# city96/ComfyUI-GGUF

Measured on NVIDIA H100. Metric: standalone dequant throughput, GGUF packed -> fp16 (algorithmic GB/s = packed bytes read + output bytes written), higher is better.
Workload: dtype f16

## Files before the change

### comfyui-gguf_b200/csrc/api.cu

```cuda
#include <stdlib.h>

#include "blocks.cuh"
#include "fallback.cuh"
#include "internal.h"

using namespace ggufb200;

static bool type_geom(int t, int *bs, int *ts)
{
    int b = 1, s = 2;
    const bool known = t == T_BF16 || with_block(t, false, [&](auto blk) {
        b = decltype(blk)::BS;
        s = decltype(blk)::TS;
        return true;
    });
    if (!known) return false;
    if (bs) *bs = b;
    if (ts) *ts = s;
    return true;
}

static bool dtype_ok(int d) { return d >= 0 && d <= 2; }
static bool aligned16(const void *p) { return (reinterpret_cast<uintptr_t>(p) & 15) == 0; }
static bool fused_type(int t) { return t != T_BF16 && type_geom(t, nullptr, nullptr); }

static int device_check()
{
    static signed char ok[64] = {};
    int dev = 0;
    if (cudaGetDevice(&dev) != cudaSuccess) {
        cudaGetLastError();
        return GGUFB200_E_CUDA;
    }
    if (dev < 0 || dev >= 64) return GGUFB200_OK;
    if (ok[dev] == 0) {
        int major = 0, minor = 0;
        if (cudaDeviceGetAttribute(&major, cudaDevAttrComputeCapabilityMajor, dev) != cudaSuccess ||
            cudaDeviceGetAttribute(&minor, cudaDevAttrComputeCapabilityMinor, dev) != cudaSuccess) {
            cudaGetLastError();
            return GGUFB200_E_CUDA;
        }
        ok[dev] = (major == 9 && minor == 0) ? 1 : -1;
    }
    return ok[dev] == 1 ? GGUFB200_OK : GGUFB200_E_DEVICE;
}

struct Route {
    int algo;
    size_t ws;
};

static LinearOptions linear_options(int flags, bool straddled)
{
    LinearOptions o;
    if (flags & GGUFB200_FLAG_GENERIC) o.producers = LinearOptions::GENERIC;
    else if (flags & GGUFB200_FLAG_EXACT_W) o.producers = LinearOptions::EXACT;
    if (flags & GGUFB200_FLAG_TILE384) o.tile = 384;
    else if (flags & GGUFB200_FLAG_TILE192) o.tile = 192;
    o.nosplit = (flags & GGUFB200_FLAG_NOSPLIT) != 0 || straddled;
    return o;
}

static Route pick_route(int type, const void *W, long long M, long long N, long long K, int act, int math, int algo_flags,
                        const LinearOptions &opt, size_t ws_avail, bool have_spans = false)
{
    const int algo = algo_flags & GGUFB200_ALGO_MASK;
    const int flags = algo_flags & ~GGUFB200_ALGO_MASK;
    const size_t dense = (size_t)N * (size_t)K * 2;
    const bool w_ok = !W || aligned16(W);
    int bs = 1;
    type_geom(type, &bs, nullptr);
    const bool straddled = straddled_rows(bs, N, K);
    const bool fusable = fused_type(type) && math == kF16 && (K % 64) == 0 && (N % 8) == 0 && !straddled;
    Route r{algo, 0};
    if (algo == GGUFB200_ALGO_AUTO) {
        const bool tmem_ok = w_ok && fused_type(type) && math == kF16 && (N % 8) == 0 && (have_spans || fused_tmem_supported(type, W, N, K));
        const bool exact = (flags & GGUFB200_FLAG_EXACT_W) != 0 || math != kF16;
        if (!w_ok) r.algo = GGUFB200_ALGO_DEQUANT_MMA;
        else if (straddled) r.algo = GGUFB200_ALGO_DEQUANT_MMA;
        else if (M <= gemv_max_m() && !exact && gemv2_supported(type, W ? W : (const void *)16, N, K, M)) r.algo = GGUFB200_ALGO_GEMV_FAST;
        else if (M <= gemv_max_m()) r.algo = GGUFB200_ALGO_GEMV;
        else if (tmem_ok) r.algo = GGUFB200_ALGO_FUSED_TMEM;
        else if (fusable && ws_avail < dense) r.algo = GGUFB200_ALGO_FUSED_MMA;
        else r.algo = GGUFB200_ALGO_DEQUANT_MMA;
    }
    switch (r.algo) {
    case GGUFB200_ALGO_DEQUANT_MMA: r.ws = dense; break;
    case GGUFB200_ALGO_FUSED_MMA: r.ws = fusable ? fused_mma_workspace(M, N, K, opt) : 0; break;
    case GGUFB200_ALGO_FUSED_TMEM: r.ws = fused_tmem_workspace(M, N, K, opt); break;
    default: r.ws = 0;
    }
    (void)act;
    return r;
}

extern "C" {

int ggufb200_version(void) { return GGUFB200_VERSION; }

const char *ggufb200_strerror(int rc)
{
    switch (rc) {
    case GGUFB200_OK: return "ok";
    case GGUFB200_E_TYPE: return "unsupported ggml quantization type (no CPU fallback is provided)";
    case GGUFB200_E_DTYPE: return "dtype code must be 0 (float16), 1 (bfloat16) or 2 (float32)";
    case GGUFB200_E_ALIGN: return "output / activation pointers must be 16-byte aligned";
    case GGUFB200_E_SHAPE: return "bad shape: sizes must be non-negative, K a multiple of the block size (or of 8 with N*K a multiple of a 256-element block), ld >= row length";
    case GGUFB200_E_NULL: return "required pointer is NULL";
    case GGUFB200_E_CUDA: return "CUDA launch failed";
    case GGUFB200_E_WORKSPACE: return "workspace too small (see ggufb200_linear_workspace)";
    case GGUFB200_E_UNSUPPORTED: return "operation not implemented for this type / dtype / shape combination";
    case GGUFB200_E_DEVICE: return "current CUDA device is not sm_90 (H100)";
// ... 349 lines not shown
```

### comfyui-gguf_b200/csrc/dequant.cu

```cuda
#include <type_traits>

#include "blocks.cuh"
#include "fallback.cuh"
#include "internal.h"
#include "wgmma.cuh"

namespace ggufb200 {

constexpr int kThreads = 128;

int g_dequant_pdl = 1;

__device__ __forceinline__ void st_otile_v4(uint32_t saddr, uint32_t a, uint32_t b, uint32_t c, uint32_t d)
{
    asm volatile("st.shared.v4.b32 [%0], {%1, %2, %3, %4};" ::"r"(saddr), "r"(a), "r"(b), "r"(c), "r"(d));
}

template <class Q, int MATH, int OUT>
__device__ __forceinline__ void dequant_tile(const uint8_t *tile, uint8_t *otile, int tile_elems, int tid)
{
    constexpr int OB = OutT<OUT>::bytes;
    constexpr int EPC = 16 / OB;
    constexpr int CH = 32 / EPC;
    const int blk_in_tile = (tid * 32) / Q::BS;
    const int e0 = (tid * 32) % Q::BS;
    if constexpr (IsFallback<Q>::value) {
        static_assert(MATH == kF32, "the fallback formats are decoded in fp32 only");
        if (tid * 32 < tile_elems) {
            float v[32];
            Q::run32(tile + blk_in_tile * Q::TS, e0, v);
            const uint32_t obase = smem_u32(otile) + tid * (32 * OB);
            const uint32_t sw = (obase >> 7) & (CH - 1);
#pragma unroll
            for (int c = 0; c < CH; ++c) {
                const float *f = v + c * EPC;
                const uint32_t oaddr = obase + ((uint32_t)c ^ sw) * 16;
                if constexpr (OUT == kF32) {
                    st_otile_v4(oaddr, __float_as_uint(f[0]), __float_as_uint(f[1]), __float_as_uint(f[2]), __float_as_uint(f[3]));
                } else {
                    st_otile_v4(oaddr, pack16<OUT, kF32>(make_float2(f[0], f[1])), pack16<OUT, kF32>(make_float2(f[2], f[3])),
                                pack16<OUT, kF32>(make_float2(f[4], f[5])), pack16<OUT, kF32>(make_float2(f[6], f[7])));
                }
            }
        }
    } else {
        constexpr int GROUP = GroupOf<Q>::value;
        if (tid * 32 < tile_elems) {
            const uint8_t *blk = tile + blk_in_tile * Q::TS;
            const GroupScale<MATH> g0 = group_scale<Q, MATH>(blk, e0);
            GroupScale<MATH> g1 = g0;
            if constexpr (GROUP == 16) g1 = group_scale<Q, MATH>(blk, e0 + 16);
            const uint32_t obase = smem_u32(otile) + tid * (32 * OB);
            const uint32_t sw = (obase >> 7) & (CH - 1);
#pragma unroll
            for (int c = 0; c < CH; ++c) {
                const int e = e0 + c * EPC;
                const bool second = (GROUP == 16) && (c * EPC >= 16);
                typename Math<MATH>::T2 v[EPC / 2];
                dequant_elems<Q, MATH, EPC>(blk, e, second ? g1 : g0, v);
                const uint32_t oaddr = obase + ((uint32_t)c ^ sw) * 16;
                if constexpr (OUT == kF32) {
                    float2 f0 = Math<MATH>::to_f32x2(v[0]), f1 = Math<MATH>::to_f32x2(v[1]);
// ... 468 lines not shown
```

### comfyui-gguf_b200/csrc/internal.h

```cpp
#pragma once
#include <cuda_runtime.h>
#include <stddef.h>
#include <stdint.h>

#include "../../include/ggufb200.h"

namespace ggufb200 {

extern int g_dequant_pdl;
extern int g_gemv2_ctas;

int dequant_dispatch(int type, const void *packed, long long n_blocks, void *out, int out_dtype, int math_dtype, cudaStream_t st, bool stable = false);
int fallback_dispatch(int type, const void *packed, long long n_blocks, void *out, int out_dtype, cudaStream_t st, bool stable);
int unpack_dispatch(int type, const void *packed, long long n_blocks, int16_t *q, int16_t *sc, int16_t *mn, cudaStream_t st);
int rows_dispatch(int type, const void *packed, long long n_table_rows, long long K, const long long *rows, long long n_rows, void *out,
                  int out_dtype, int math_dtype, cudaStream_t st);
constexpr int kKronMaxPatches = 8;
int dequant_kron_dispatch(int type, const void *packed, long long N, long long K, void *out, int out_dtype, int math_dtype,
                          const ggufb200_kron_patch *patches, int n_patches, cudaStream_t st, bool stable);
constexpr int kLowrankMaxPatches = GGUFB200_LOWRANK_MAX_PATCHES;
int dequant_lowrank_dispatch(int type, const void *packed, long long N, long long K, void *out, int out_dtype, int math_dtype,
                             const ggufb200_lowrank_patch *patches, int n_patches, cudaStream_t st);

int gemv_max_m();
int gemv_dispatch(int type, const void *W, long long N, long long K, const void *X, long long M, long long ldx, int act_dtype, int math_dtype,
                  const void *bias, int bias_dtype, void *Y, long long ldy, cudaStream_t st);
bool gemv2_supported(int type, const void *W, long long N, long long K, long long M);
int gemv2_dispatch(int type, const void *W, long long N, long long K, const void *X, long long M, long long ldx, int act_dtype, const void *bias,
                   int bias_dtype, void *Y, long long ldy, cudaStream_t st, bool w_stable = false);

inline bool straddled_rows(int block_size, long long N, long long K)
{
    return block_size == 256 && K % 256 != 0 && (N * K) % 256 == 0;
}

size_t repack_bytes(int type, long long N, long long K, int *pitch, long long *span_stride);
int repack_dispatch(int type, const void *W, long long N, long long K, void *out, cudaStream_t st);

struct LinearOptions {
    enum Producers { FAST, EXACT, GENERIC };
    Producers producers = FAST;
    int tile = 0;
    bool nosplit = false;
};

int dense_gemm(const void *W, long long N, long long K, long long ldw, const void *X, long long M, long long ldx, int act_dtype,
               const void *bias, int bias_dtype, void *Y, long long ldy, cudaStream_t st, const float *scale = nullptr);
size_t fused_mma_workspace(long long M, long long N, long long K, const LinearOptions &opt);
void fused_mma_plan(long long M, long long N, long long K, size_t ws_bytes, const LinearOptions &opt, int *tile_rows, int *splits,
                    int *kb_per_split, int *ctas);
int fused_mma_linear(int type, const void *W, long long N, long long K, const void *X, long long M, long long ldx, int act_dtype,
                     const void *bias, int bias_dtype, void *Y, long long ldy, void *ws, size_t ws_bytes, const LinearOptions &opt,
                     cudaStream_t st);
constexpr int kLoraMaxKblocks = 8;
struct LoraOperands {
    const void *T;
    long long ldt;
    const void *U;
    long long ldu;
    int kblocks;
    const int32_t *tiles;
};
bool fused_tmem_supported(int type, const void *W, long long N, long long K);
size_t fused_tmem_workspace(long long M, long long N, long long K, const LinearOptions &opt);
void fused_tmem_plan(long long M, long long N, long long K, size_t ws_bytes, const LinearOptions &opt, int *tile_tokens, int *splits,
                     int *spans_per_split, int *items);
int fused_tmem_linear(int type, const void *W, const void *Wspan, long long span_stride, long long N, long long K, const void *X, long long M,
                      long long ldx, int act_dtype, const void *bias, int bias_dtype, void *Y, long long ldy, void *ws, size_t ws_bytes,
                      const LinearOptions &opt, const LoraOperands &lora, cudaStream_t st, const float *scale = nullptr);

int scale_columns_dispatch(const void *X, long long M, long long K, long long ldx, int act_dtype, const float *col_scale, void *Y,
                           long long ldy, cudaStream_t st);

}
```

### comfyui-gguf_b200/csrc/linear_sm90.cu

```cuda
#include "internal.h"
#include "linear_sm90.cuh"

namespace ggufb200 {

constexpr size_t kSplitWsCap = 24u << 20;
constexpr int kSpan = 256;

static size_t split_ws(size_t ws_bytes) { return ws_bytes > kSplitWsCap ? kSplitWsCap : ws_bytes; }

struct KRanges {
    long long per, count;
};
static KRanges k_ranges(long long spans, long long s)
{
    const long long per = (spans + s - 1) / s;
    return {per, (spans + per - 1) / per};
}

static size_t partial_bytes(int splits, long long M, long long N) { return splits > 1 ? (size_t)splits * (size_t)M * (size_t)N * 4 : 0; }

template <int ACT, int BN, bool SCALED>
static int dense_launch(const void *W, long long N, long long K, long long ldw, const void *X, long long M, long long ldx, const void *bias,
                        int bias_dtype, void *Y, long long ldy, cudaStream_t st, const float *scale)
{
// ... 150 lines not shown
            if (r.count != s) continue;
            const int per = (int)r.per, splits = (int)r.count;
            const long long items = tiles * splits;
            const long long ctas = items * 2 * cands[c].accs;
            const long long rounds = (ctas + sms - 1) / sms;
            const double t_kb = 4.0 * cands[c].tt > 2000.0 ? 4.0 * cands[c].tt : 2000.0;
            double cost = (double)rounds * (4.0 * per * t_kb + 3000.0);
            if (splits > 1) cost += (double)(splits + 1) * (double)slice / (16.0 * sms) + 6000.0;
            if (best.n_items == 0 || cost < best_cost * 0.98) {
                best_cost = cost;
                best.tt = cands[c].tt; best.accs = cands[c].accs; best.splits = splits; best.spans_per_split = per;
                best.ttiles = ttiles; best.ftiles = ftiles; best.n_items = (int)items;
            }
        }
    }
    return best;
}

size_t fused_tmem_workspace(long long M, long long N, long long K, const LinearOptions &opt)
{
    return partial_bytes(tmem_plan(M, N, K, kSplitWsCap, opt.tile, !opt.nosplit).splits, M, N);
}

void fused_tmem_plan(long long M, long long N, long long K, size_t ws_bytes, const LinearOptions &opt, int *tile_tokens, int *splits,
                     int *spans_per_split, int *items)
{
    const TmemPlan pl = tmem_plan(M, N, K, ws_bytes, opt.tile, !opt.nosplit);
    *tile_tokens = pl.tt * pl.accs;
    *splits = pl.splits;
    *spans_per_split = pl.spans_per_split;
    *items = pl.n_items;
}

struct TmemArgs {
    const void *W;
    const void *Wspan;
    long long span_stride;
    long long N, K;
    const void *X;
    long long M, ldx;
    const void *bias;
    int bias_dtype;
    void *Y;
    long long ldy;
    void *ws;
    size_t ws_bytes;
    const LinearOptions &opt;
    const LoraOperands &lora;
    cudaStream_t st;
    bool straddled;
    const float *scale;
};

template <class Q, class Prod, int ACT, int TT, bool SCALED>
static int tmem_launch(const TmemArgs &a, const TmemPlan &pl, float *partial)
{
    CUtensorMap tmX, tmT;
    if (!make_kblock_map(&tmX, a.X, a.M, a.K, a.ldx, ACT, TT)) return GGUFB200_E_CUDA;
    tmT = tmX;
    if (a.lora.T && !make_kblock_map(&tmT, a.lora.T, a.M, (long long)kBlockK * a.lora.kblocks, a.lora.ldt, ACT, TT)) return GGUFB200_E_CUDA;
    WgParams p{};
    p.M = a.M; p.N = a.N; p.K = a.K;
    p.bias = partial ? nullptr : a.bias;
    p.bias_dtype = a.bias_dtype;
    p.Y = reinterpret_cast<uint8_t *>(a.Y);
    p.ldy = a.ldy;
    p.partial = partial;
    p.W = reinterpret_cast<const uint8_t *>(a.W);
    if (a.straddled) {
        p.Wspan = reinterpret_cast<const uint8_t *>(a.Wspan ? a.Wspan : a.W);
        p.span_stride = a.Wspan ? a.span_stride : Q::TS;
    } else {
        p.row_bytes = a.K / Q::BS * Q::TS;
        p.Wspan = reinterpret_cast<const uint8_t *>(a.Wspan);
        p.span_stride = a.span_stride;
    }
    p.loraU = a.lora.T ? reinterpret_cast<const uint16_t *>(a.lora.U) : nullptr;
    p.ldu = a.lora.ldu;
    p.lora_kb = a.lora.kblocks;
    p.lora_tiles = a.lora.tiles;
    p.scale = partial ? nullptr : a.scale;
    p.ftiles = 2 * pl.ftiles;
    p.ttiles = pl.ttiles * pl.accs;
    p.kb_per_split = 4 * pl.spans_per_split;
    p.kb_total = a.straddled ? (int)(a.K / kBlockK) : 4 * (int)((a.K + kSpan - 1) / kSpan);
    if constexpr (Q::BS == 256) {
        if (a.straddled) return wg_launch<Q, Prod, ACT, TT, true, true, SCALED>(tmX, tmX, tmT, p, pl.splits, a.st);
    }
    return wg_launch<Q, Prod, ACT, TT, true, false, SCALED>(tmX, tmX, tmT, p, pl.splits, a.st);
}

template <class Q, class Prod, int ACT, bool SCALED> static int tmem_tiles(const TmemArgs &a, const TmemPlan &pl, float *partial)
{
    if (pl.tt == 32) return tmem_launch<Q, Prod, ACT, 32, SCALED>(a, pl, partial);
    if (pl.tt == 128) return tmem_launch<Q, Prod, ACT, 128, SCALED>(a, pl, partial);
    return tmem_launch<Q, Prod, ACT, 192, SCALED>(a, pl, partial);
}

template <class Q> struct FmaMatters {
    static constexpr bool value = Q::TS == 144 || Q::TS == 176;
};

template <class Q, int ACT, bool SCALED> static int tmem_run(const TmemArgs &a)
{
    const TmemPlan pl = tmem_plan(a.M, a.N, a.K, a.ws_bytes, a.opt.tile, !a.opt.nosplit);
    float *partial = pl.splits > 1 ? reinterpret_cast<float *>(a.ws) : nullptr;
    int rc;
    if constexpr (!FastProducer<Q>::fast) {
        rc = tmem_tiles<Q, Producer<Q>, ACT, SCALED>(a, pl, partial);
    } else if (a.opt.producers == LinearOptions::GENERIC) {
        rc = tmem_tiles<Q, Producer<Q>, ACT, SCALED>(a, pl, partial);
    } else if constexpr (FmaMatters<Q>::value) {
        rc = a.opt.producers == LinearOptions::EXACT ? tmem_tiles<Q, FastProducer<Q, false>, ACT, SCALED>(a, pl, partial)
                                                     : tmem_tiles<Q, FastProducer<Q, true>, ACT, SCALED>(a, pl, partial);
    } else {
        rc = tmem_tiles<Q, FastProducer<Q, true>, ACT, SCALED>(a, pl, partial);
    }
    if (rc != GGUFB200_OK || !partial) return rc;
    return wg_finalize<ACT, SCALED>(partial, pl.splits, a.bias, a.bias_dtype, a.Y, a.M, a.N, a.ldy, a.st, a.scale);
}

template <class Q> static bool canonical_ok(const void *W, long long N, long long K)
{
    const bool aligned = SpanOf<Q>::BYTES % 16 == 0 && K % kBlockK == 0 && (reinterpret_cast<uintptr_t>(W) & 15) == 0;
    if (straddled_rows(Q::BS, N, K)) return aligned;
    return aligned && (K / Q::BS * Q::TS) % 16 == 0;
}

bool fused_tmem_supported(int type, const void *W, long long N, long long K)
{
    if (N % 8 != 0 || K % 8 != 0) return false;
    return with_block(type, false, [&](auto blk) { return canonical_ok<decltype(blk)>(W, N, K); });
}

int fused_tmem_linear(int type, const void *W, const void *Wspan, long long span_stride, long long N, long long K, const void *X, long long M,
                      long long ldx, int act_dtype, const void *bias, int bias_dtype, void *Y, long long ldy, void *ws, size_t ws_bytes,
                      const LinearOptions &opt, const LoraOperands &lora, cudaStream_t st, const float *scale)
{
    if (N % 8 != 0 || K % 8 != 0) return GGUFB200_E_UNSUPPORTED;
    return with_block(type, GGUFB200_E_UNSUPPORTED, [&](auto blk) {
        using Q = decltype(blk);
        const bool straddled = straddled_rows(Q::BS, N, K);
// ... 10 lines not shown
```

### comfyui-gguf_b200/csrc/linear_sm90.cuh

```cuda
#pragma once
#include <type_traits>

#include "produce.cuh"
#include "wgmma.cuh"

namespace ggufb200 {

constexpr int kWgThreads = 384;

struct WgParams {
    long long M, N, K;
    const void *bias;
    int bias_dtype;
    uint8_t *Y;
    long long ldy;
    float *partial;
    const uint8_t *W;
    long long row_bytes;
    const uint8_t *Wspan;
    long long span_stride;
    const uint16_t *loraU;
    int ttiles, ftiles;
    int kb_per_split, kb_total;
    long long ldu;
    int lora_kb;
    const int *lora_tiles;
    const float *scale;
};

template <int TN, bool TRANS> struct WgCfg {
    static constexpr int TOK = TRANS ? TN : 128;
    static constexpr int FEAT = TRANS ? 128 : TN;
    static constexpr int A_BYTES = 128 * 128;
    static constexpr int B_BYTES = TN * 128;
    static constexpr int STAGE = A_BYTES + B_BYTES;
    static constexpr int RAW_STAGES = (227 * 1024 - 2048) / STAGE;
    static constexpr int STAGES = RAW_STAGES > 8 ? 8 : RAW_STAGES;
    static constexpr int YPITCH = FEAT * 2 + 16;
    static constexpr int SMEM = STAGES * STAGE + 1024 + 256;
    static_assert(TOK * YPITCH <= STAGES * STAGE, "epilogue staging reuses the operand ring");
    static_assert(B_BYTES % 1024 == 0, "swizzled tiles need 1024-byte alignment");
};

template <int ACT> __device__ __forceinline__ uint32_t wg_h2_to_act(uint32_t h)
{
    if constexpr (ACT == kBF16) {
        const float2 f = __half22float2(*reinterpret_cast<const __half2 *>(&h));
        const __nv_bfloat162 b = __floats2bfloat162_rn(f.x, f.y);
        return *reinterpret_cast<const uint32_t *>(&b);
    } else {
        return h;
    }
}

template <class Q, class Prod, int ACT, int TN, bool TRANS, bool STRADDLED = false, bool SCALED = false>
__global__ void __launch_bounds__(kWgThreads, 1)
wg_linear_kernel(const __grid_constant__ CUtensorMap tmX, const __grid_constant__ CUtensorMap tmW, const __grid_constant__ CUtensorMap tmT,
                 const WgParams p)
{
    using Cfg = WgCfg<TN, TRANS>;
    constexpr bool DENSE = std::is_same<Prod, void>::value;
    constexpr int STAGES = Cfg::STAGES, TOK = Cfg::TOK, FEAT = Cfg::FEAT;
    constexpr int WROWS = TRANS ? 128 : TN;

    const int per = p.ftiles * p.ttiles;
    const int split = blockIdx.x / per;
    const int rem = blockIdx.x - split * per;
    const long long feat0 = (long long)(rem / p.ttiles) * FEAT;
    const long long tok0 = (long long)(rem % p.ttiles) * TOK;
    if (tok0 >= p.M || feat0 >= p.N) return;
    const int kb0 = split * p.kb_per_split;
    const int nkb_main = min(p.kb_per_split, p.kb_total - kb0);
    int lora_first = 0, lora_n = 0;
    if (p.loraU != nullptr && split == 0) {
        lora_n = p.lora_kb;
        if (p.lora_tiles) {
            const long long ft = feat0 / 128;
            lora_first = min(max(p.lora_tiles[2 * ft], 0), p.lora_kb);
            lora_n = min(max(p.lora_tiles[2 * ft + 1], 0), p.lora_kb - lora_first);
        }
    }
    const int nkb = nkb_main + lora_n;

    extern __shared__ uint8_t wg_smem_raw[];
    uint8_t *tiles = reinterpret_cast<uint8_t *>((reinterpret_cast<uintptr_t>(wg_smem_raw) + 1023) & ~(uintptr_t)1023);
    uint64_t *full = reinterpret_cast<uint64_t *>(tiles + STAGES * Cfg::STAGE);
    uint64_t *empty = full + STAGES;

    const int wg = threadIdx.x >> 7;
    const int t = threadIdx.x & 127;
    if (threadIdx.x == 0) {
        for (int s = 0; s < STAGES; ++s) {
            mbar_init(&full[s], DENSE ? 1 : 1 + 4);
            mbar_init(&empty[s], 256);
        }
        fence_mbar_init();
    }
    __syncthreads();

    if (wg == 0) {
        for (int i = 0; i < nkb; ++i) {
            const int s = i % STAGES;
            mbar_wait(&empty[s], (uint32_t)(((i / STAGES) & 1) ^ 1));
            uint8_t *a_tile = tiles + s * Cfg::STAGE;
            uint8_t *b_tile = a_tile + Cfg::A_BYTES;
            uint8_t *x_tile = TRANS ? b_tile : a_tile;
            uint8_t *w_tile = TRANS ? a_tile : b_tile;
            const int kb = kb0 + i;
            const bool lora_kb = i >= nkb_main;
            const int lj = lora_first + i - nkb_main;
            if (t == 0) {
                mbar_arrive_expect_tx(&full[s], TOK * 128 + (DENSE ? WROWS * 128 : 0));
                tma_load_2d(x_tile, lora_kb ? &tmT : &tmX, &full[s], lora_kb ? lj * kBlockK : kb * kBlockK, (int)tok0);
                if constexpr (DENSE) tma_load_2d(w_tile, &tmW, &full[s], kb * kBlockK, (int)feat0);
            }
            if constexpr (!DENSE) {
#pragma unroll 1
                for (int r = t; r < WROWS; r += 128) {
                    const long long n = feat0 + r;
                    const uint32_t dst = smem_u32(w_tile) + (uint32_t)r * 128;
                    auto emit = [&](int half, const uint32_t (&o)[16]) {
#pragma unroll
                        for (int c = 0; c < 4; ++c) {
                            const int chunk = half * 4 + c;
                            st_shared_v4(dst + (uint32_t)((chunk ^ (r & 7)) << 4), wg_h2_to_act<ACT>(o[4 * c]), wg_h2_to_act<ACT>(o[4 * c + 1]),
                                         wg_h2_to_act<ACT>(o[4 * c + 2]), wg_h2_to_act<ACT>(o[4 * c + 3]));
                        }
                    };
                    if (n >= p.N || (!lora_kb && (long long)kb * kBlockK >= p.K)) {
#pragma unroll
                        for (int c = 0; c < 8; ++c) st_shared_v4(dst + (uint32_t)(c << 4), 0, 0, 0, 0);
                    } else if (lora_kb) {
                        const uint4 *urow = reinterpret_cast<const uint4 *>(p.loraU + n * p.ldu + lj * kBlockK);
#pragma unroll
                        for (int half = 0; half < 2; ++half) {
                            uint32_t o[16];
#pragma unroll
                            for (int q = 0; q < 4; ++q) {
                                const uint4 v = urow[half * 4 + q];
                                o[4 * q] = v.x; o[4 * q + 1] = v.y; o[4 * q + 2] = v.z; o[4 * q + 3] = v.w;
                            }
                            emit(half, o);
                        }
                    } else if constexpr (STRADDLED) {
                        static_assert(TRANS && Q::BS == 256, "straddled rows: FUSED_TMEM, 256-element blocks");
                        const long long e = n * p.K + (long long)kb * kBlockK;
                        Prod::run64(p.Wspan + (e >> 8) * p.span_stride, (int)(e >> 6) & 3, emit);
                    } else {
                        const int span = kb >> 2;
                        const uint8_t *src = p.Wspan ? p.Wspan + (long long)span * p.span_stride + n * SpanOf<Q>::PITCH
                                                     : p.W + n * p.row_bytes + (long long)span * SpanOf<Q>::BYTES;
                        Prod::run64(src, kb & 3, emit);
                    }
                }
                fence_proxy_async_smem();
                __syncwarp();
                if ((t & 31) == 0) mbar_arrive(&full[s]);
            }
        }
        return;
    }

    const int cw = wg - 1;
    constexpr int NR = TN / 2;
    float acc[NR];
#pragma unroll
    for (int j = 0; j < NR; ++j) acc[j] = 0.f;
    const uint32_t base = smem_u32(tiles);
    for (int i = 0; i < nkb; ++i) {
        const int s = i % STAGES;
        mbar_wait(&full[s], (uint32_t)((i / STAGES) & 1));
        const uint32_t a_addr = base + (uint32_t)(s * Cfg::STAGE) + (uint32_t)(cw * 64 * 128);
        const uint32_t b_addr = base + (uint32_t)(s * Cfg::STAGE + Cfg::A_BYTES);
        const uint64_t da = wg_desc_sw128(a_addr), db = wg_desc_sw128(b_addr);
        wgmma_fence();
#pragma unroll
        for (int j = 0; j < kBlockK / 16; ++j) Wgmma<ACT, TN>::mma(acc, da + (uint64_t)(2 * j), db + (uint64_t)(2 * j));
        wgmma_commit();
        if (i > 0) {
            wgmma_wait<1>();
            mbar_arrive(&empty[(i - 1) % STAGES]);
        }
    }
    wgmma_wait<0>();

    const int warp = (threadIdx.x >> 5) & 3, lane = threadIdx.x & 31;
    const int arow0 = cw * 64 + warp * 16 + (lane >> 2);
    const int bcol0 = 2 * (lane & 3);
    if (p.partial) {
        float *P = p.partial + (long long)split * p.M * p.N;
#pragma unroll
        for (int j = 0; j < NR / 4; ++j)
#pragma unroll
            for (int h = 0; h < 2; ++h)
#pragma unroll
                for (int e = 0; e < 2; ++e) {
                    const int ar = arow0 + 8 * h, bc = 8 * j + bcol0 + e;
                    const long long tok = tok0 + (TRANS ? bc : ar), f = feat0 + (TRANS ? ar : bc);
                    if (tok < p.M && f < p.N) P[tok * p.N + f] = acc[4 * j + 2 * h + e];
                }
        return;
    }
    asm volatile("bar.sync 1, 256;" ::: "memory");
    const uint32_t ystage = base;
#pragma unroll
    for (int j = 0; j < NR / 4; ++j)
#pragma unroll
        for (int h = 0; h < 2; ++h)
#pragma unroll
            for (int e = 0; e < 2; ++e) {
                const int ar = arow0 + 8 * h, bc = 8 * j + bcol0 + e;
                const int tk = TRANS ? bc : ar, f = TRANS ? ar : bc;
                float v = acc[4 * j + 2 * h + e];
                if constexpr (SCALED) {
                    if (feat0 + f < p.N) v *= p.scale[feat0 + f];
                }
                if (p.bias && feat0 + f < p.N) v += wg_bias<ACT>(p.bias, p.bias_dtype, feat0 + f);
                uint16_t hb;
                if constexpr (ACT == kBF16) hb = __bfloat16_as_ushort(__float2bfloat16_rn(v));
                else hb = __half_as_ushort(__float2half_rn(v));
                asm volatile("st.shared.u16 [%0], %1;" ::"r"(ystage + (uint32_t)(tk * Cfg::YPITCH + f * 2)), "h"(hb) : "memory");
            }
    asm volatile("bar.sync 1, 256;" ::: "memory");
    constexpr int CPR = FEAT / 8;
    for (int c = threadIdx.x - 128; c < TOK * CPR; c += 256) {
        const int tk = c / CPR, f = (c % CPR) * 8;
        const long long m = tok0 + tk, n = feat0 + f;
        if (m < p.M && n < p.N) {
            uint32_t a, b, cc, d;
            asm volatile("ld.shared.v4.b32 {%0, %1, %2, %3}, [%4];" : "=r"(a), "=r"(b), "=r"(cc), "=r"(d) : "r"(ystage + (uint32_t)(tk * Cfg::YPITCH + f * 2)));
            st_global_v4(p.Y + (m * p.ldy + n) * 2, a, b, cc, d);
        }
    }
}

template <class Q, class Prod, int ACT, int TN, bool TRANS, bool STRADDLED = false, bool SCALED = false>
static int wg_launch(const CUtensorMap &tmX, const CUtensorMap &tmW, const CUtensorMap &tmT, const WgParams &p, int splits, cudaStream_t st)
{
    using Cfg = WgCfg<TN, TRANS>;
    auto kern = wg_linear_kernel<Q, Prod, ACT, TN, TRANS, STRADDLED, SCALED>;
    static unsigned char attr[64] = {};
    if (!ensure_dynamic_smem(kern, Cfg::SMEM, attr)) return GGUFB200_E_CUDA;
    const long long ctas = (long long)p.ftiles * p.ttiles * splits;
    if (ctas <= 0 || ctas > 0x7fffffffll) return GGUFB200_E_SHAPE;
    kern<<<(unsigned)ctas, kWgThreads, Cfg::SMEM, st>>>(tmX, tmW, tmT, p);
    return cudaGetLastError() == cudaSuccess ? GGUFB200_OK : GGUFB200_E_CUDA;
}

template <int ACT, bool SCALED = false>
__global__ void __launch_bounds__(256) wg_finalize_kernel(const float *__restrict__ P, int splits, const void *__restrict__ bias, int bias_dtype,
                                                          uint8_t *__restrict__ Y, long long M, long long N, long long ldy,
                                                          const float *__restrict__ scale)
{
    const long long n8 = N / 8;
    for (long long i = (long long)blockIdx.x * 256 + threadIdx.x; i < M * n8; i += (long long)gridDim.x * 256) {
        const long long m = i / n8, n = (i % n8) * 8;
        float v[8] = {0.f, 0.f, 0.f, 0.f, 0.f, 0.f, 0.f, 0.f};
        for (int sp = 0; sp < splits; ++sp) {
            const float *src = P + ((long long)sp * M + m) * N + n;
            const float4 a = *reinterpret_cast<const float4 *>(src), b = *reinterpret_cast<const float4 *>(src + 4);
            v[0] += a.x; v[1] += a.y; v[2] += a.z; v[3] += a.w;
            v[4] += b.x; v[5] += b.y; v[6] += b.z; v[7] += b.w;
        }
        if constexpr (SCALED) {
            const float4 a = *reinterpret_cast<const float4 *>(scale + n), b = *reinterpret_cast<const float4 *>(scale + n + 4);
            v[0] *= a.x; v[1] *= a.y; v[2] *= a.z; v[3] *= a.w;
            v[4] *= b.x; v[5] *= b.y; v[6] *= b.z; v[7] *= b.w;
        }
        if (bias) {
#pragma unroll
            for (int j = 0; j < 8; ++j) v[j] += wg_bias<ACT>(bias, bias_dtype, n + j);
        }
        st_global_v4(Y + (m * ldy + n) * 2, wg_pack<ACT>(v[0], v[1]), wg_pack<ACT>(v[2], v[3]), wg_pack<ACT>(v[4], v[5]), wg_pack<ACT>(v[6], v[7]));
    }
}

template <int ACT, bool SCALED = false>
static int wg_finalize(const float *P, int splits, const void *bias, int bias_dtype, void *Y, long long M, long long N, long long ldy, cudaStream_t st,
                       const float *scale = nullptr)
{
    const long long work = M * (N / 8);
    const long long cap = (long long)sm_count() * 8;
    const unsigned grid = (unsigned)((work + 255) / 256 < cap ? (work + 255) / 256 : cap);
    wg_finalize_kernel<ACT, SCALED><<<grid, 256, 0, st>>>(P, splits, bias, bias_dtype, reinterpret_cast<uint8_t *>(Y), M, N, ldy, scale);
    return cudaGetLastError() == cudaSuccess ? GGUFB200_OK : GGUFB200_E_CUDA;
}

}
```

### comfyui-gguf_b200/csrc/produce.cuh

```cuda
#pragma once
#include "blocks.cuh"

namespace ggufb200 {

template <class Q> struct SpanOf {
    static constexpr int BYTES = (256 / Q::BS) * Q::TS;
    static constexpr int PAD16 = (BYTES + 15) / 16 * 16;
    static constexpr int PITCH = BYTES % 16 == 0 ? BYTES : ((PAD16 / 16) % 2 == 1 ? PAD16 : PAD16 + 16);
};

GG_HD uint4 ld_span16(const uint8_t *p)
{
#ifdef __CUDA_ARCH__
    return __ldg(reinterpret_cast<const uint4 *>(p));
#else
    return *reinterpret_cast<const uint4 *>(p);
#endif
}
GG_HD uint32_t ld_span4(const uint8_t *p)
{
#ifdef __CUDA_ARCH__
    return __ldg(reinterpret_cast<const unsigned int *>(p));
#else
    return *reinterpret_cast<const uint32_t *>(p);
#endif
}

GG_HD uint32_t h2_bits(__half2 v) { return *reinterpret_cast<uint32_t *>(&v); }
GG_HD __half2 bits_h2(uint32_t v) { return *reinterpret_cast<__half2 *>(&v); }

template <class Q> struct Producer {
    static constexpr bool fast = false;
    template <class Emit> static GG_HD void run64(const uint8_t *span, int kq, Emit &&emit)
    {
        constexpr int GROUP = GroupOf<Q>::value;
#pragma unroll
        for (int half = 0; half < 2; ++half) {
            const int k = kq * 64 + half * 32;
            const uint8_t *blk = span + (k / Q::BS) * Q::TS;
            const int e0 = k % Q::BS;
            const GroupScale<kF16> g0 = group_scale<Q, kF16>(blk, e0);
            GroupScale<kF16> g1 = g0;
            if constexpr (GROUP == 16) g1 = group_scale<Q, kF16>(blk, e0 + 16);
            uint32_t o[16];
#pragma unroll
            for (int c = 0; c < 4; ++c) {
                __half2 v[4];
                dequant_elems<Q, kF16, 8>(blk, e0 + c * 8, (GROUP == 16 && c >= 2) ? g1 : g0, v);
#pragma unroll
                for (int j = 0; j < 4; ++j) o[4 * c + j] = h2_bits(v[j]);
            }
            emit(half, o);
        }
    }
};

template <class Q, bool FMA = true> struct FastProducer : Producer<Q> {};



GG_HD __half2 h2_fma(__half2 a, __half2 b, __half2 c)
{
#ifdef __CUDA_ARCH__
    return __hfma2(a, b, c);
#else
    const float2 fa = __half22float2(a), fb = __half22float2(b), fc = __half22float2(c);
    const double x = (double)fa.x * (double)fb.x + (double)fc.x, y = (double)fa.y * (double)fb.y + (double)fc.y;
    return __halves2half2(__double2half(x), __double2half(y));
#endif
}

template <bool FMA> GG_HD __half2 k_step(__half2 q, __half2 D, __half2 nM)
{
    if constexpr (FMA) return h2_fma(q, D, nM);
    else return __hadd2_rn(__hmul2_rn(D, q), nM);
}

GG_HD __half2 k_dm(uint32_t dm_bits, uint32_t sc, uint32_t mn)
{
    const __half2 k1024 = __half2half2(__ushort_as_half((unsigned short)0x6400u));
    const __half2 scm = __hsub2_rn(bits_h2((sc & 0xFFu) | ((mn & 0xFFu) << 16) | 0x64006400u), k1024);
    return __hmul2_rn(bits_h2(dm_bits), scm);
}

GG_HD void k_scale_pair(uint32_t w0, uint32_t w1, uint32_t w2, int kq, uint32_t &sc, uint32_t &mn)
{
    const int sh = 16 * (kq & 1);
    const uint32_t a = (w0 >> sh) & 0xFFFFu, b = (w1 >> sh) & 0xFFFFu, c = (w2 >> sh) & 0xFFFFu;
    if (kq < 2) {
        sc = a & 0x3F3Fu;
        mn = b & 0x3F3Fu;
    } else {
        sc = (c & 0x0F0Fu) | ((a >> 2) & 0x3030u);
        mn = ((c >> 4) & 0x0F0Fu) | ((b >> 2) & 0x3030u);
    }
}

template <bool HIGH> GG_HD void bytes_to_h2(uint32_t v, __half2 &lo, __half2 &hi)
{
    const uint32_t magic = HIGH ? 0x54545454u : 0x64646464u;
    const __half2 off = __half2half2(__ushort_as_half((unsigned short)(HIGH ? 0x5400u : 0x6400u)));
    lo = __hsub2_rn(bits_h2(prmt(v, magic, 0x4140u)), off);
    hi = __hsub2_rn(bits_h2(prmt(v, magic, 0x4342u)), off);
}

template <bool FMA> struct FastProducer<Block<T_Q4_K>, FMA> {
    static constexpr bool fast = true;
    template <class Emit> static GG_HD void run64(const uint8_t *blk, int kq, Emit &&emit)
    {
        const uint4 h = ld_span16(blk);
        const uint4 qa = ld_span16(blk + 16 + 32 * kq);
        const uint4 qb = ld_span16(blk + 32 + 32 * kq);
        uint32_t sc, mn;
        k_scale_pair(h.y, h.z, h.w, kq, sc, mn);
        const __half2 dm0 = k_dm(h.x, sc, mn), dm1 = k_dm(h.x, sc >> 8, mn >> 8);
        const uint32_t w[8] = {qa.x, qa.y, qa.z, qa.w, qb.x, qb.y, qb.z, qb.w};
        {
            const __half2 D = __low2half2(dm0), nM = __hneg2(__high2half2(dm0));
            uint32_t o[16];
#pragma unroll
            for (int i = 0; i < 8; ++i) {
                __half2 a, b;
                bytes_to_h2<false>(w[i] & 0x0F0F0F0Fu, a, b);
                o[2 * i] = h2_bits(k_step<FMA>(a, D, nM));
                o[2 * i + 1] = h2_bits(k_step<FMA>(b, D, nM));
            }
            emit(0, o);
        }
        {
            const __half2 D = __low2half2(dm1), nM = __hneg2(__high2half2(dm1));
            uint32_t o[16];
#pragma unroll
            for (int i = 0; i < 8; ++i) {
                __half2 a, b;
                bytes_to_h2<true>(w[i] & 0xF0F0F0F0u, a, b);
                o[2 * i] = h2_bits(k_step<FMA>(a, D, nM));
                o[2 * i + 1] = h2_bits(k_step<FMA>(b, D, nM));
            }
            emit(1, o);
        }
    }
};

template <bool FMA> struct FastProducer<Block<T_Q5_K>, FMA> {
    static constexpr bool fast = true;
    template <class Emit> static GG_HD void run64(const uint8_t *blk, int kq, Emit &&emit)
    {
        const uint4 h = ld_span16(blk);
        const uint4 ha = ld_span16(blk + 16), hb = ld_span16(blk + 32);
        const uint4 qa = ld_span16(blk + 48 + 32 * kq);
        const uint4 qb = ld_span16(blk + 64 + 32 * kq);
        uint32_t sc, mn;
        k_scale_pair(h.y, h.z, h.w, kq, sc, mn);
        const __half2 dm0 = k_dm(h.x, sc, mn), dm1 = k_dm(h.x, sc >> 8, mn >> 8);
        const uint32_t w[8] = {qa.x, qa.y, qa.z, qa.w, qb.x, qb.y, qb.z, qb.w};
        const uint32_t qh[8] = {ha.x, ha.y, ha.z, ha.w, hb.x, hb.y, hb.z, hb.w};
#pragma unroll
        for (int half = 0; half < 2; ++half) {
            const __half2 dm = half ? dm1 : dm0;
            const __half2 D = __low2half2(dm), nM = __hneg2(__high2half2(dm));
            const int sb = 2 * kq + half;
            uint32_t o[16];
#pragma unroll
            for (int i = 0; i < 8; ++i) {
                const uint32_t lo = (half ? (w[i] >> 4) : w[i]) & 0x0F0F0F0Fu;
                const uint32_t u = lo | (((qh[i] >> sb) & 0x01010101u) << 4);
                __half2 a, b;
                bytes_to_h2<false>(u, a, b);
                o[2 * i] = h2_bits(k_step<FMA>(a, D, nM));
                o[2 * i + 1] = h2_bits(k_step<FMA>(b, D, nM));
            }
            emit(half, o);
        }
    }
};

template <bool FMA> struct FastProducer<Block<T_Q8_0>, FMA> {
    static constexpr bool fast = true;
    template <class Emit> static GG_HD void run64(const uint8_t *span, int kq, Emit &&emit)
    {
        const __half2 k1152 = __half2half2(__ushort_as_half((unsigned short)(0x6400u + 128u)));
#pragma unroll
        for (int half = 0; half < 2; ++half) {
            const uint8_t *p = span + 68 * kq + (half ? 32 : 0);
            uint32_t o[16];
            if (half == 0) {
                uint32_t wd[9];
#pragma unroll
                for (int i = 0; i < 9; ++i) wd[i] = ld_span4(p + 4 * i);
                const __half2 D = __half2half2(__ushort_as_half((unsigned short)(wd[0] & 0xFFFFu)));
#pragma unroll
                for (int i = 0; i < 9; ++i) wd[i] ^= 0x80808080u;
#pragma unroll
                for (int j = 0; j < 16; ++j) {
                    const int byte = 2 + 2 * j;
                    const uint32_t sel = (byte & 2) ? 0x4342u : 0x4140u;
                    const __half2 x = __hsub2_rn(bits_h2(prmt(wd[byte >> 2], 0x64646464u, sel)), k1152);
                    o[j] = h2_bits(__hmul2_rn(D, x));
                }
            } else {
                uint32_t wd[9];
#pragma unroll
                for (int i = 0; i < 9; ++i) wd[i] = ld_span4(p + 4 * i);
                const __half2 D = __half2half2(__ushort_as_half((unsigned short)(wd[0] >> 16)));
#pragma unroll
                for (int i = 1; i < 9; ++i) wd[i] ^= 0x80808080u;
#pragma unroll
                for (int j = 0; j < 16; ++j) {
                    const int byte = 4 + 2 * j;
                    const uint32_t sel = (byte & 2) ? 0x4342u : 0x4140u;
                    const __half2 x = __hsub2_rn(bits_h2(prmt(wd[byte >> 2], 0x64646464u, sel)), k1152);
                    o[j] = h2_bits(__hmul2_rn(D, x));
                }
            }
            emit(half, o);
        }
    }
};

template <bool FMA> struct FastProducer<Block<T_Q4_0>, FMA> {
    static constexpr bool fast = true;
    template <class Emit> static GG_HD void run64(const uint8_t *span, int kq, Emit &&emit)
    {
        uint32_t wd[9];
#pragma unroll
        for (int i = 0; i < 9; ++i) wd[i] = ld_span4(span + 36 * kq + 4 * i);
        const __half2 k1032 = __half2half2(__ushort_as_half((unsigned short)(0x6400u + 8u)));
        const __half2 k72 = __half2half2(__ushort_as_half((unsigned short)0x5480u));
#pragma unroll
        for (int half = 0; half < 2; ++half) {
            const int base = 18 * half;
            const uint32_t dbits = (wd[base >> 2] >> (8 * (base & 3))) & 0xFFFFu;
            const __half2 D = __half2half2(__ushort_as_half((unsigned short)dbits));
            uint32_t o[16];
#pragma unroll
            for (int j = 0; j < 8; ++j) {
                const int byte = base + 2 + 2 * j;
                const uint32_t sel = (byte & 2) ? 0x4342u : 0x4140u;
                const uint32_t word = wd[byte >> 2];
                const __half2 lo = __hsub2_rn(bits_h2(prmt(word & 0x0F0F0F0Fu, 0x64646464u, sel)), k1032);
                const __half2 hi = __hsub2_rn(bits_h2(prmt(word & 0xF0F0F0F0u, 0x54545454u, sel)), k72);
                o[j] = h2_bits(__hmul2_rn(D, lo));
                o[8 + j] = h2_bits(__hmul2_rn(D, hi));
            }
            emit(half, o);
        }
    }
};

template <bool FMA> struct FastProducer<Block<T_Q6_K>, FMA> {
    static constexpr bool fast = true;
    template <class Emit> static GG_HD void run64(const uint8_t *blk, int kq, Emit &&emit)
    {
        const int hh = kq >> 1, up = kq & 1;
        const uint8_t *ql = blk + 64 * hh;
        const uint4 h0 = ld_span16(blk + 128 + 32 * hh), h1 = ld_span16(blk + 144 + 32 * hh);
        const uint32_t hw[8] = {h0.x, h0.y, h0.z, h0.w, h1.x, h1.y, h1.z, h1.w};
        const uint32_t sw = ld_span4(blk + 192 + 4 * kq);
        const __half d = __ushort_as_half((unsigned short)(ld_span4(blk + 208) & 0xFFFFu));
        const __half2 k1056 = __half2half2(__ushort_as_half((unsigned short)(0x6400u + 32u)));
#pragma unroll
        for (int half = 0; half < 2; ++half) {
            const uint4 l0 = ld_span16(ql + 32 * half), l1 = ld_span16(ql + 32 * half + 16);
            const uint32_t lw[8] = {l0.x, l0.y, l0.z, l0.w, l1.x, l1.y, l1.z, l1.w};
            const int s0 = (int)(int8_t)(sw >> (16 * half)), s1 = (int)(int8_t)(sw >> (16 * half + 8));
            const __half2 D0 = __half2half2(__hmul_rn(d, __int2half_rn(s0))), D1 = __half2half2(__hmul_rn(d, __int2half_rn(s1)));
            const int fsh = 2 * (2 * up + half);
            uint32_t o[16];
#pragma unroll
            for (int i = 0; i < 8; ++i) {
                const uint32_t lo = (up ? (lw[i] >> 4) : lw[i]) & 0x0F0F0F0Fu;
                const uint32_t u = lo | (((hw[i] >> fsh) & 0x03030303u) << 4);
                const __half2 D = i < 4 ? D0 : D1;
                o[2 * i] = h2_bits(__hmul2_rn(D, __hsub2_rn(bits_h2(prmt(u, 0x64646464u, 0x4140u)), k1056)));
                o[2 * i + 1] = h2_bits(__hmul2_rn(D, __hsub2_rn(bits_h2(prmt(u, 0x64646464u, 0x4342u)), k1056)));
            }
            emit(half, o);
        }
    }
};

}
```

Before: 2887.

## Stage weight spans into shared memory via TMA in fused linear kernel

Adds a double-buffered shared-memory ring in the sm90 fused linear kernel: one thread loads each packed weight span with TMA or a bulk copy, and the producers decode from shared memory instead of global. The aim is to overlap weight fetches with decode and avoid scattered global loads, at the cost of fewer operand stages and extra mbarrier waits. It also doubles the standalone dequant kernel's block size from 128 to 256 threads, which is the only part that touches the measured dequant path.

```diff
diff --git a/comfyui-gguf_b200/csrc/api.cu b/comfyui-gguf_b200/csrc/api.cu
--- a/comfyui-gguf_b200/csrc/api.cu
+++ b/comfyui-gguf_b200/csrc/api.cu
@@ -58,6 +58,7 @@
     if (flags & GGUFB200_FLAG_TILE384) o.tile = 384;
     else if (flags & GGUFB200_FLAG_TILE192) o.tile = 192;
     o.nosplit = (flags & GGUFB200_FLAG_NOSPLIT) != 0 || straddled;
+    o.unstaged = (flags & GGUFB200_FLAG_UNSTAGED) != 0;
     return o;
 }
 
diff --git a/comfyui-gguf_b200/csrc/dequant.cu b/comfyui-gguf_b200/csrc/dequant.cu
--- a/comfyui-gguf_b200/csrc/dequant.cu
+++ b/comfyui-gguf_b200/csrc/dequant.cu
@@ -7,7 +7,7 @@
 
 namespace ggufb200 {
 
-constexpr int kThreads = 128;
+constexpr int kThreads = 256;
 
 int g_dequant_pdl = 1;
 
diff --git a/comfyui-gguf_b200/csrc/internal.h b/comfyui-gguf_b200/csrc/internal.h
--- a/comfyui-gguf_b200/csrc/internal.h
+++ b/comfyui-gguf_b200/csrc/internal.h
@@ -42,6 +42,7 @@
     Producers producers = FAST;
     int tile = 0;
     bool nosplit = false;
+    bool unstaged = false;
 };
 
 int dense_gemm(const void *W, long long N, long long K, long long ldw, const void *X, long long M, long long ldx, int act_dtype,
diff --git a/comfyui-gguf_b200/csrc/linear_sm90.cu b/comfyui-gguf_b200/csrc/linear_sm90.cu
--- a/comfyui-gguf_b200/csrc/linear_sm90.cu
+++ b/comfyui-gguf_b200/csrc/linear_sm90.cu
@@ -226,12 +226,27 @@
     const float *scale;
 };
 
+template <class Q> static bool make_span_map(CUtensorMap *tm, const void *W, long long N, long long row_bytes)
+{
+    TensorMapEncodeFn fn = tensor_map_encode_fn();
+    if (!fn) return false;
+    cuuint64_t dims[2] = {(cuuint64_t)(row_bytes / 4), (cuuint64_t)N};
+    cuuint64_t strides[1] = {(cuuint64_t)row_bytes};
+    cuuint32_t box[2] = {(cuuint32_t)(SpanOf<Q>::BYTES / 4), 128};
+    cuuint32_t estr[2] = {1, 1};
+    return fn(tm, CU_TENSOR_MAP_DATA_TYPE_UINT32, 2, const_cast<void *>(W), dims, strides, box, estr, CU_TENSOR_MAP_INTERLEAVE_NONE,
+              CU_TENSOR_MAP_SWIZZLE_NONE, CU_TENSOR_MAP_L2_PROMOTION_L2_256B, CU_TENSOR_MAP_FLOAT_OOB_FILL_NONE) == CUDA_SUCCESS;
+}
+
 template <class Q, class Prod, int ACT, int TT, bool SCALED>
 static int tmem_launch(const TmemArgs &a, const TmemPlan &pl, float *partial)
 {
-    CUtensorMap tmX, tmT;
+    CUtensorMap tmX, tmT, tmS;
     if (!make_kblock_map(&tmX, a.X, a.M, a.K, a.ldx, ACT, TT)) return GGUFB200_E_CUDA;
     tmT = tmX;
+    tmS = tmX;
+    const bool stage = !a.straddled && !a.opt.unstaged;
+    if (stage && !a.Wspan && !make_span_map<Q>(&tmS, a.W, a.N, a.K / Q::BS * Q::TS)) return GGUFB200_E_CUDA;
     if (a.lora.T && !make_kblock_map(&tmT, a.lora.T, a.M, (long long)kBlockK * a.lora.kblocks, a.lora.ldt, ACT, TT)) return GGUFB200_E_CUDA;
     WgParams p{};
     p.M = a.M; p.N = a.N; p.K = a.K;
@@ -258,10 +273,11 @@
     p.ttiles = pl.ttiles * pl.accs;
     p.kb_per_split = 4 * pl.spans_per_split;
     p.kb_total = a.straddled ? (int)(a.K / kBlockK) : 4 * (int)((a.K + kSpan - 1) / kSpan);
+    p.stage_spans = stage ? 1 : 0;
     if constexpr (Q::BS == 256) {
         if (a.straddled) return wg_launch<Q, Prod, ACT, TT, true, true, SCALED>(tmX, tmX, tmT, p, pl.splits, a.st);
     }
-    return wg_launch<Q, Prod, ACT, TT, true, false, SCALED>(tmX, tmX, tmT, p, pl.splits, a.st);
+    return wg_launch<Q, Prod, ACT, TT, true, false, SCALED>(tmX, tmS, tmT, p, pl.splits, a.st);
 }
 
 template <class Q, class Prod, int ACT, bool SCALED> static int tmem_tiles(const TmemArgs &a, const TmemPlan &pl, float *partial)
diff --git a/comfyui-gguf_b200/csrc/linear_sm90.cuh b/comfyui-gguf_b200/csrc/linear_sm90.cuh
--- a/comfyui-gguf_b200/csrc/linear_sm90.cuh
+++ b/comfyui-gguf_b200/csrc/linear_sm90.cuh
@@ -26,18 +26,35 @@
     int lora_kb;
     const int *lora_tiles;
     const float *scale;
+    int stage_spans;
 };
 
-template <int TN, bool TRANS> struct WgCfg {
+constexpr int kSpanBufs = 2;
+
+template <class Q, bool ON> struct SpanGeom {
+    static constexpr int BYTES = 0, PITCH = 0;
+};
+template <class Q> struct SpanGeom<Q, true> : SpanOf<Q> {};
+template <class Q, class Prod, bool TRANS, bool STRADDLED> struct WgSpans {
+    static constexpr bool ON = TRANS && !STRADDLED && !std::is_same<Prod, void>::value;
+    static constexpr int BYTES = SpanGeom<Q, ON>::BYTES;
+    static constexpr int PITCH = SpanGeom<Q, ON>::PITCH;
+    static constexpr int BUF = 128 * PITCH;
+    static constexpr int RING = ON ? kSpanBufs * BUF : 0;
+    static_assert(BUF % 128 == 0, "span buffers must stay 128-byte aligned for the TMA engine");
+};
+
+template <int TN, bool TRANS, int RING = 0> struct WgCfg {
     static constexpr int TOK = TRANS ? TN : 128;
     static constexpr int FEAT = TRANS ? 128 : TN;
     static constexpr int A_BYTES = 128 * 128;
     static constexpr int B_BYTES = TN * 128;
     static constexpr int STAGE = A_BYTES + B_BYTES;
-    static constexpr int RAW_STAGES = (227 * 1024 - 2048) / STAGE;
+    static constexpr int RAW_STAGES = (227 * 1024 - 2048 - RING) / STAGE;
     static constexpr int STAGES = RAW_STAGES > 8 ? 8 : RAW_STAGES;
     static constexpr int YPITCH = FEAT * 2 + 16;
-    static constexpr int SMEM = STAGES * STAGE + 1024 + 256;
+    static constexpr int SMEM = STAGES * STAGE + RING + 1024 + 256;
+    static_assert(STAGES >= 2, "the operand ring needs two stages");
     static_assert(TOK * YPITCH <= STAGES * STAGE, "epilogue staging reuses the operand ring");
     static_assert(B_BYTES % 1024 == 0, "swizzled tiles need 1024-byte alignment");
 };
@@ -58,7 +75,8 @@
 wg_linear_kernel(const __grid_constant__ CUtensorMap tmX, const __grid_constant__ CUtensorMap tmW, const __grid_constant__ CUtensorMap tmT,
                  const WgParams p)
 {
-    using Cfg = WgCfg<TN, TRANS>;
+    using SP = WgSpans<Q, Prod, TRANS, STRADDLED>;
+    using Cfg = WgCfg<TN, TRANS, SP::RING>;
     constexpr bool DENSE = std::is_same<Prod, void>::value;
     constexpr int STAGES = Cfg::STAGES, TOK = Cfg::TOK, FEAT = Cfg::FEAT;
     constexpr int WROWS = TRANS ? 128 : TN;
@@ -81,11 +99,16 @@
         }
     }
     const int nkb = nkb_main + lora_n;
+    const bool stage = SP::ON && p.stage_spans != 0;
+    const int nspans = nkb_main >> 2;
 
     extern __shared__ uint8_t wg_smem_raw[];
     uint8_t *tiles = reinterpret_cast<uint8_t *>((reinterpret_cast<uintptr_t>(wg_smem_raw) + 1023) & ~(uintptr_t)1023);
-    uint64_t *full = reinterpret_cast<uint64_t *>(tiles + STAGES * Cfg::STAGE);
+    uint8_t *ring = tiles + STAGES * Cfg::STAGE;
+    uint64_t *full = reinterpret_cast<uint64_t *>(ring + SP::RING);
     uint64_t *empty = full + STAGES;
+    uint64_t *sfull = empty + STAGES;
+    uint64_t *sempty = sfull + kSpanBufs;
 
     const int wg = threadIdx.x >> 7;
     const int t = threadIdx.x & 127;
@@ -94,13 +117,39 @@
             mbar_init(&full[s], DENSE ? 1 : 1 + 4);
             mbar_init(&empty[s], 256);
         }
+        if constexpr (SP::ON) {
+            for (int b = 0; b < kSpanBufs; ++b) {
+                mbar_init(&sfull[b], 1);
+                mbar_init(&sempty[b], 4);
+            }
+        }
         fence_mbar_init();
     }
     __syncthreads();
 
     if (wg == 0) {
+        auto stage_span = [&](int j) {
+            uint64_t *bar = &sfull[j % kSpanBufs];
+            uint8_t *dst = ring + (j % kSpanBufs) * SP::BUF;
+            const int span = (kb0 >> 2) + j;
+            mbar_arrive_expect_tx(bar, SP::BUF);
+            if (p.Wspan) bulk_g2s(dst, p.Wspan + (long long)span * p.span_stride + feat0 * SP::PITCH, SP::BUF, bar);
+            else tma_load_2d(dst, &tmW, bar, span * (SP::BYTES / 4), (int)feat0);
+        };
+        if constexpr (SP::ON) {
+            if (stage && t == 0)
+                for (int j = 0; j < kSpanBufs - 1 && j < nspans; ++j) stage_span(j);
+        }
         for (int i = 0; i < nkb; ++i) {
             const int s = i % STAGES;
+            const bool span_start = stage && i < nkb_main && (i & 3) == 0;
+            if constexpr (SP::ON) {
+                const int j = i >> 2;
+                if (span_start && t == 0 && j + kSpanBufs - 1 < nspans) {
+                    if (j >= 1) mbar_wait(&sempty[(j - 1) % kSpanBufs], (uint32_t)(((j - 1) / kSpanBufs) & 1));
+                    stage_span(j + kSpanBufs - 1);
+                }
+            }
             mbar_wait(&empty[s], (uint32_t)(((i / STAGES) & 1) ^ 1));
             uint8_t *a_tile = tiles + s * Cfg::STAGE;
             uint8_t *b_tile = a_tile + Cfg::A_BYTES;
@@ -114,6 +163,9 @@
                 tma_load_2d(x_tile, lora_kb ? &tmT : &tmX, &full[s], lora_kb ? lj * kBlockK : kb * kBlockK, (int)tok0);
                 if constexpr (DENSE) tma_load_2d(w_tile, &tmW, &full[s], kb * kBlockK, (int)feat0);
             }
+            if constexpr (SP::ON) {
+                if (span_start) mbar_wait(&sfull[(i >> 2) % kSpanBufs], (uint32_t)(((i >> 2) / kSpanBufs) & 1));
+            }
             if constexpr (!DENSE) {
 #pragma unroll 1
                 for (int r = t; r < WROWS; r += 128) {
@@ -146,6 +198,8 @@
                         static_assert(TRANS && Q::BS == 256, "straddled rows: FUSED_TMEM, 256-element blocks");
                         const long long e = n * p.K + (long long)kb * kBlockK;
                         Prod::run64(p.Wspan + (e >> 8) * p.span_stride, (int)(e >> 6) & 3, emit);
+                    } else if (SP::ON && stage) {
+                        Prod::template run64<LdShared>(ring + ((i >> 2) % kSpanBufs) * SP::BUF + r * SP::PITCH, kb & 3, emit);
                     } else {
                         const int span = kb >> 2;
                         const uint8_t *src = p.Wspan ? p.Wspan + (long long)span * p.span_stride + n * SpanOf<Q>::PITCH
@@ -155,7 +209,10 @@
                 }
                 fence_proxy_async_smem();
                 __syncwarp();
-                if ((t & 31) == 0) mbar_arrive(&full[s]);
+                if ((t & 31) == 0) {
+                    mbar_arrive(&full[s]);
+                    if (stage && i < nkb_main && (i & 3) == 3) mbar_arrive(&sempty[(i >> 2) % kSpanBufs]);
+                }
             }
         }
         return;
@@ -237,7 +294,7 @@
 template <class Q, class Prod, int ACT, int TN, bool TRANS, bool STRADDLED = false, bool SCALED = false>
 static int wg_launch(const CUtensorMap &tmX, const CUtensorMap &tmW, const CUtensorMap &tmT, const WgParams &p, int splits, cudaStream_t st)
 {
-    using Cfg = WgCfg<TN, TRANS>;
+    using Cfg = WgCfg<TN, TRANS, WgSpans<Q, Prod, TRANS, STRADDLED>::RING>;
     auto kern = wg_linear_kernel<Q, Prod, ACT, TN, TRANS, STRADDLED, SCALED>;
     static unsigned char attr[64] = {};
     if (!ensure_dynamic_smem(kern, Cfg::SMEM, attr)) return GGUFB200_E_CUDA;
diff --git a/comfyui-gguf_b200/csrc/produce.cuh b/comfyui-gguf_b200/csrc/produce.cuh
--- a/comfyui-gguf_b200/csrc/produce.cuh
+++ b/comfyui-gguf_b200/csrc/produce.cuh
@@ -26,12 +26,39 @@
 #endif
 }
 
+struct LdGlobal {
+    static GG_HD uint4 v16(const uint8_t *p) { return ld_span16(p); }
+    static GG_HD uint32_t v4(const uint8_t *p) { return ld_span4(p); }
+};
+struct LdShared {
+    static GG_HD uint4 v16(const uint8_t *p)
+    {
+#ifdef __CUDA_ARCH__
+        uint4 v;
+        asm volatile("ld.shared.v4.b32 {%0, %1, %2, %3}, [%4];" : "=r"(v.x), "=r"(v.y), "=r"(v.z), "=r"(v.w) : "r"((uint32_t)__cvta_generic_to_shared(p)));
+        return v;
+#else
+        return *reinterpret_cast<const uint4 *>(p);
+#endif
+    }
+    static GG_HD uint32_t v4(const uint8_t *p)
+    {
+#ifdef __CUDA_ARCH__
+        uint32_t v;
+        asm volatile("ld.shared.b32 %0, [%1];" : "=r"(v) : "r"((uint32_t)__cvta_generic_to_shared(p)));
+        return v;
+#else
+        return *reinterpret_cast<const uint32_t *>(p);
+#endif
+    }
+};
+
 GG_HD uint32_t h2_bits(__half2 v) { return *reinterpret_cast<uint32_t *>(&v); }
 GG_HD __half2 bits_h2(uint32_t v) { return *reinterpret_cast<__half2 *>(&v); }
 
 template <class Q> struct Producer {
     static constexpr bool fast = false;
-    template <class Emit> static GG_HD void run64(const uint8_t *span, int kq, Emit &&emit)
+    template <class Ld = LdGlobal, class Emit> static GG_HD void run64(const uint8_t *span, int kq, Emit &&emit)
     {
         constexpr int GROUP = GroupOf<Q>::value;
 #pragma unroll
@@ -106,11 +133,11 @@
 
 template <bool FMA> struct FastProducer<Block<T_Q4_K>, FMA> {
     static constexpr bool fast = true;
-    template <class Emit> static GG_HD void run64(const uint8_t *blk, int kq, Emit &&emit)
-    {
-        const uint4 h = ld_span16(blk);
-        const uint4 qa = ld_span16(blk + 16 + 32 * kq);
-        const uint4 qb = ld_span16(blk + 32 + 32 * kq);
+    template <class Ld = LdGlobal, class Emit> static GG_HD void run64(const uint8_t *blk, int kq, Emit &&emit)
+    {
+        const uint4 h = Ld::v16(blk);
+        const uint4 qa = Ld::v16(blk + 16 + 32 * kq);
+        const uint4 qb = Ld::v16(blk + 32 + 32 * kq);
         uint32_t sc, mn;
         k_scale_pair(h.y, h.z, h.w, kq, sc, mn);
         const __half2 dm0 = k_dm(h.x, sc, mn), dm1 = k_dm(h.x, sc >> 8, mn >> 8);
@@ -144,12 +171,12 @@
 
 template <bool FMA> struct FastProducer<Block<T_Q5_K>, FMA> {
     static constexpr bool fast = true;
-    template <class Emit> static GG_HD void run64(const uint8_t *blk, int kq, Emit &&emit)
-    {
-        const uint4 h = ld_span16(blk);
-        const uint4 ha = ld_span16(blk + 16), hb = ld_span16(blk + 32);
-        const uint4 qa = ld_span16(blk + 48 + 32 * kq);
-        const uint4 qb = ld_span16(blk + 64 + 32 * kq);
+    template <class Ld = LdGlobal, class Emit> static GG_HD void run64(const uint8_t *blk, int kq, Emit &&emit)
+    {
+        const uint4 h = Ld::v16(blk);
+        const uint4 ha = Ld::v16(blk + 16), hb = Ld::v16(blk + 32);
+        const uint4 qa = Ld::v16(blk + 48 + 32 * kq);
+        const uint4 qb = Ld::v16(blk + 64 + 32 * kq);
         uint32_t sc, mn;
         k_scale_pair(h.y, h.z, h.w, kq, sc, mn);
         const __half2 dm0 = k_dm(h.x, sc, mn), dm1 = k_dm(h.x, sc >> 8, mn >> 8);
@@ -177,7 +204,7 @@
 
 template <bool FMA> struct FastProducer<Block<T_Q8_0>, FMA> {
     static constexpr bool fast = true;
-    template <class Emit> static GG_HD void run64(const uint8_t *span, int kq, Emit &&emit)
+    template <class Ld = LdGlobal, class Emit> static GG_HD void run64(const uint8_t *span, int kq, Emit &&emit)
     {
         const __half2 k1152 = __half2half2(__ushort_as_half((unsigned short)(0x6400u + 128u)));
 #pragma unroll
@@ -187,7 +214,7 @@
             if (half == 0) {
                 uint32_t wd[9];
 #pragma unroll
-                for (int i = 0; i < 9; ++i) wd[i] = ld_span4(p + 4 * i);
+                for (int i = 0; i < 9; ++i) wd[i] = Ld::v4(p + 4 * i);
                 const __half2 D = __half2half2(__ushort_as_half((unsigned short)(wd[0] & 0xFFFFu)));
 #pragma unroll
                 for (int i = 0; i < 9; ++i) wd[i] ^= 0x80808080u;
@@ -201,7 +228,7 @@
             } else {
                 uint32_t wd[9];
 #pragma unroll
-                for (int i = 0; i < 9; ++i) wd[i] = ld_span4(p + 4 * i);
+                for (int i = 0; i < 9; ++i) wd[i] = Ld::v4(p + 4 * i);
                 const __half2 D = __half2half2(__ushort_as_half((unsigned short)(wd[0] >> 16)));
 #pragma unroll
                 for (int i = 1; i < 9; ++i) wd[i] ^= 0x80808080u;
@@ -220,11 +247,11 @@
 
 template <bool FMA> struct FastProducer<Block<T_Q4_0>, FMA> {
     static constexpr bool fast = true;
-    template <class Emit> static GG_HD void run64(const uint8_t *span, int kq, Emit &&emit)
+    template <class Ld = LdGlobal, class Emit> static GG_HD void run64(const uint8_t *span, int kq, Emit &&emit)
     {
         uint32_t wd[9];
 #pragma unroll
-        for (int i = 0; i < 9; ++i) wd[i] = ld_span4(span + 36 * kq + 4 * i);
+        for (int i = 0; i < 9; ++i) wd[i] = Ld::v4(span + 36 * kq + 4 * i);
         const __half2 k1032 = __half2half2(__ushort_as_half((unsigned short)(0x6400u + 8u)));
         const __half2 k72 = __half2half2(__ushort_as_half((unsigned short)0x5480u));
 #pragma unroll
@@ -250,18 +277,18 @@
 
 template <bool FMA> struct FastProducer<Block<T_Q6_K>, FMA> {
     static constexpr bool fast = true;
-    template <class Emit> static GG_HD void run64(const uint8_t *blk, int kq, Emit &&emit)
+    template <class Ld = LdGlobal, class Emit> static GG_HD void run64(const uint8_t *blk, int kq, Emit &&emit)
     {
         const int hh = kq >> 1, up = kq & 1;
         const uint8_t *ql = blk + 64 * hh;
-        const uint4 h0 = ld_span16(blk + 128 + 32 * hh), h1 = ld_span16(blk + 144 + 32 * hh);
+        const uint4 h0 = Ld::v16(blk + 128 + 32 * hh), h1 = Ld::v16(blk + 144 + 32 * hh);
         const uint32_t hw[8] = {h0.x, h0.y, h0.z, h0.w, h1.x, h1.y, h1.z, h1.w};
-        const uint32_t sw = ld_span4(blk + 192 + 4 * kq);
-        const __half d = __ushort_as_half((unsigned short)(ld_span4(blk + 208) & 0xFFFFu));
+        const uint32_t sw = Ld::v4(blk + 192 + 4 * kq);
+        const __half d = __ushort_as_half((unsigned short)(Ld::v4(blk + 208) & 0xFFFFu));
         const __half2 k1056 = __half2half2(__ushort_as_half((unsigned short)(0x6400u + 32u)));
 #pragma unroll
         for (int half = 0; half < 2; ++half) {
-            const uint4 l0 = ld_span16(ql + 32 * half), l1 = ld_span16(ql + 32 * half + 16);
+            const uint4 l0 = Ld::v16(ql + 32 * half), l1 = Ld::v16(ql + 32 * half + 16);
             const uint32_t lw[8] = {l0.x, l0.y, l0.z, l0.w, l1.x, l1.y, l1.z, l1.w};
             const int s0 = (int)(int8_t)(sw >> (16 * half)), s1 = (int)(int8_t)(sw >> (16 * half + 8));
             const __half2 D0 = __half2half2(__hmul_rn(d, __int2half_rn(s0))), D1 = __half2half2(__hmul_rn(d, __int2half_rn(s1)));
```

Result: no change. 2904, median of 6 (+0.6%).
